# mfkiwl/erlangnetwork-gnsslib-sdr

Hardware: AMD Instinct MI355X
Metric: correlations/sec (1 ms coh) + x real-time, 32-SV L1CA @16.368 Msps (higher is better)
Workload: dtype int8 samples x int8 carrier LUT -> int32 accumulators (exact); NCOs: the reference's fp64 running sums, bit for bit; 1 GPU; BASELINE configs[2]: 32-SV GPS L1CA tracking, 5-tap E/P/L correlators (CORRN=2, CORRD=3), 1 ms coherent, 16.368 Msps int8 IQ, per GPU; channels_per_gpu=32, epochs_per_launch=1000, taps=5, loop=open (frequencies held per launch); see closed_loop (--full), if_broadcast=none (1 GPU)

## Files before the change

erlangnetwork-gnsslib-sdr_amd/csrc/gnsscorr_nco.h:

```cpp
#pragma once

#include <math.h>
#include <stdint.h>
#include <string.h>
#include <type_traits>

#if defined(__HIPCC__)
#define GC_HD __host__ __device__ inline
#define GC_HDM __host__ __device__
#define GC_HD_NOINLINE __host__ __device__ __attribute__((noinline))
#else
#define GC_HD static inline
#define GC_HDM
#define GC_HD_NOINLINE static
#endif
#if defined(__clang__)
#define GC_FP_STRICT _Pragma("clang fp contract(off)")
#else
#define GC_FP_STRICT
#endif

#if defined(__HIP_DEVICE_COMPILE__)
#define GC_DDIV(a, b) __ddiv_rn((a), (b))
#else
// ... 1483 lines not shown
}

GC_HD bool gc_carrier_value_step_one(const GcCarPlan &P, const GcCarStepC &C, double remcarr, int n, int kprem,
                                     double *remcarr_out)
{
    GC_FP_STRICT
    if (C.ex0 == GC_NO_TABLE || n < 1) return false;
    double x = gc_div_y(remcarr * GC_NCO_CDIV, GC_NCO_DPI, P.ydpi);
    if (!gc_one_binade_walk(x, C.s, n, &x)) return false;
    bool held;
    const double p = gc_prem_checked(x, kprem, &held);
    if (!held) return false;
    *remcarr_out = p;
    return true;
}
```

erlangnetwork-gnsslib-sdr_amd/csrc/gnsscorr_plan.hip:

```cpp
#include <cstdlib>
#include <cstddef>
#include <hip/hip_runtime.h>

#include "gnsscorr_internal.h"

namespace {


#define GC_SPEC_WC  9.313225746154785e-10
#define GC_SPEC_WK  9.313225746154785e-10

struct SpecChan {
    GcCodePlan PC;
    GcCarPlan PK;
    GcCarStepC CK;
    double ci, spc, ps, dlen;
    int clen, smax;
    int tmax;
    bool ok;
};

__device__ __forceinline__ void spec_chan_init(SpecChan &C, const GcChan &c, const GcTrkState &s, bool with_prem)
{
    C.ci = __dmul_rn(c.ti, s.codefreq);
// ... 40 lines not shown
            if (!gc_carrier_claims_step<true>(C.PK, C.CK, g0, n, ck, &G)) G = gc_carrier_period_any<GcFillLoop, GcNoEmit, false>(C.PK, g0, n, fill, ne, &tier);
            dk = G - g1;
            dk = dk > 0.5 * GC_NCO_DPI ? dk - GC_NCO_DPI : (dk < -0.5 * GC_NCO_DPI ? dk + GC_NCO_DPI : dk);
            if (!(fabs(dc) < 1.0e300)) dc = 0.0;
            if (!(fabs(dk) < 1.0e300)) dk = 0.0;
        }
    }
    devc[i] = dc;
    devk[i] = dk;
}

#define GC_SPEC_CHUNK 256
__global__ __launch_bounds__(GC_SPEC_CHUNK) void trk_spec_kernel(const GcChan *__restrict__ chan, const GcTrkState *__restrict__ state_in,
                                                                  const double *__restrict__ devc, const double *__restrict__ devk,
                                                                  int *__restrict__ claims_code, int *__restrict__ claims_car,
                                                                  int nch, int nepoch, int e_off)
{
    __shared__ double shc[GC_SPEC_CHUNK], shk[GC_SPEC_CHUNK];
    const int nchunk = (nepoch + GC_SPEC_CHUNK - 1) / GC_SPEC_CHUNK;
    const int ch = blockIdx.x / nchunk, chunk = blockIdx.x - ch * nchunk, tid = threadIdx.x;
    if (ch >= nch) return;
    const int T = e_off + nepoch;
    const int eb = chunk * GC_SPEC_CHUNK + tid;
    const int e = e_off + eb;
    const int base = e_off + chunk * GC_SPEC_CHUNK;
    double pc = 0.0, pk = 0.0;
    for (int j = tid; j < base; j += GC_SPEC_CHUNK) {
        pc += devc[(size_t)ch * T + j];
        pk += devk[(size_t)ch * T + j];
    }
    shc[tid] = pc;
// ... 14 lines not shown
        shc[tid] += ac;
        shk[tid] += ak;
        __syncthreads();
    }
    if (eb >= nepoch) return;
    const double sumc = basec + (tid ? shc[tid - 1] : 0.0), sumk = basek + (tid ? shk[tid - 1] : 0.0);
    const GcTrkState s = state_in[ch];
    SpecChan C;
    spec_chan_init(C, chan[ch], s, false);
    GcCodeClaims cc;
    GcCarClaims ck;
    cc.tag = 0;
    ck.tag = 0;
    cc.n = cc.pad = 0;
    cc.lo = cc.hi = ck.lo = ck.hi = 0.0;
    if (C.ok) {
        double r0, g0;
        int nhat;
        gc_spec_start(s.remcode, s.remcarr, C.ci, C.spc, C.ps, C.dlen, e, &r0, &g0, &nhat);
        const double rt = r0 + sumc, gt = g0 + sumk;
        int ncode = 0;
        bool bracketed = false;
#pragma unroll 1
        for (int att = 0; att < 2 && !bracketed; att++) {
            const double w = att == 0 ? GC_SPEC_WC : GC_SPEC_WC * 0.00390625;
            const double lo = rt - w, hi = rt + w;
            const int nlo = gc_period_nsamp(C.dlen, lo, C.spc), nhi = gc_period_nsamp(C.dlen, hi, C.spc);
            if (!(nlo == nhi && nlo > 0 && nlo <= (1 << 24))) continue;
            double dummy;
            const bool side = (lo - C.PC.smaxci < 0.0) == (hi - C.PC.smaxci < 0.0);
            const bool oklo = gc_code_claims<true>(C.PC, lo, nlo + 2 * C.smax, cc, &dummy);
            const bool okhi = oklo && gc_code_claims<false>(C.PC, hi, nlo + 2 * C.smax, cc, &dummy);
            const bool tailfits = nlo + 2 * C.smax - cc.jsum <= C.tmax;
            if (side && oklo && okhi && tailfits) {
                bracketed = true;
                ncode = nlo;
                cc.tag = 1;
                cc.n = nlo;
                cc.lo = lo;
                cc.hi = hi;
            }
        }
        if (!bracketed) {
            ncode = gc_period_nsamp(C.dlen, rt, C.spc);
            cc.tag = 0;
            if (ncode > 0 && ncode <= (1 << 24)) {
                double dummy;
                cc.tag = (gc_code_claims<true>(C.PC, rt, ncode + 2 * C.smax, cc, &dummy) && ncode + 2 * C.smax - cc.jsum <= C.tmax) ? 3 : 0;
            }
            cc.n = ncode;
            cc.lo = cc.hi = rt;
        }
        const int nk = ncode;
        if (nk > 0 && nk <= (1 << 24)) {
            bool kbr = false;
// ... 19 lines not shown
                ck.tag = ok ? (ck.tag == 2 ? 2 : 3) : 0;
                ck.lo = ck.hi = gt;
            }
            ck.nl = nk;
        }
    }
    const size_t row = (size_t)ch * nepoch + eb;
    int4 *rc = reinterpret_cast<int4 *>(claims_code) + row * (GC_CLAIM_ROW / 4);
    int4 *rk = reinterpret_cast<int4 *>(claims_car) + row * (GC_CLAIM_ROW / 4);
    const int4 *pc4 = reinterpret_cast<const int4 *>(&cc), *pk4 = reinterpret_cast<const int4 *>(&ck);
#pragma unroll
    for (int q = 0; q < GC_CLAIM_ROW / 4; q++) {
        rc[q] = pc4[q];
        rk[q] = pk4[q];
    }
}

__device__ unsigned long long gc_plan_stats[8];

__host__ __device__ inline int plan2_class(double ti, double codefreq, int clen, int smax)
{
    const double ci = ti * codefreq;
    if (!(ci > 0.0) || !gc_fast_has_table(ci)) return -1;
    const int itop = gc_expo(gc_u2d(gc_d2u((double)clen) - 1)) - (gc_expo(ci) + 2);
    if (itop < 7 || itop > 12) return -1;
    if (smax + 1 > GC_CLAIM_TAIL2) return -1;
    return (itop - 7) * 3 + gc_tail_class(smax);
}

#define GC_PLAN_MAXE 4096
__device__ __attribute__((noinline)) void trk_plan_body(const GcChan *__restrict__ chan,
                                                        const GcTrkState *__restrict__ state_in,
                                                        GcTrkState *__restrict__ state_out,
// ... 80 lines not shown
    }
}

__global__ __launch_bounds__(128) void trk_plan_kernel(const GcChan *__restrict__ chan, const GcTrkState *__restrict__ state_in,
                                                       GcTrkState *__restrict__ state_out, GcTrkPlan *__restrict__ plan,
                                                       int nch, int nepoch)
{
    trk_plan_body(chan, state_in, state_out, plan, nch, nepoch);
}

#define GC_P4_BLK 64
struct Plan4Shared {
    int nsh[GC_PLAN_MAXE];
    double vstart[2][GC_P4_BLK];
    unsigned long long vbuff[GC_P4_BLK];
    int prog;
    GcCarPlan pkfull;
};
__shared__ __attribute__((aligned(16))) Plan4Shared g_plan4;

__device__ __forceinline__ int plan2_uni(int v) { return __builtin_amdgcn_readfirstlane(v); }
template <class T>
__device__ __forceinline__ T *plan2_uni(T *p)
{
    const uint64_t u = (uint64_t)p;
    const unsigned lo = (unsigned)__builtin_amdgcn_readfirstlane((int)(unsigned)u);
    const unsigned hi = (unsigned)__builtin_amdgcn_readfirstlane((int)(unsigned)(u >> 32));
    return (T *)(((uint64_t)hi << 32) | lo);
}
__device__ __forceinline__ double plan2_uni(double x)
// ... 7 lines not shown
#define GC_CONST __attribute__((address_space(4)))
typedef int gc_v4i __attribute__((ext_vector_type(4)));
__device__ __forceinline__ GcCodeClaims plan4_code_row(const GC_CONST gc_v4i *r)
{
    const gc_v4i v0 = r[0], v1 = r[1], v2 = r[2], v3 = r[3], v4 = r[4], v5 = r[5];
    GcCodeClaims c;
    c.tag = v0.x; c.i0 = v0.y; c.q = v0.z; c.nl = v0.w;
    c.jsum = v1.x; c.dm[0] = v1.y; c.dm[1] = v1.z; c.dm[2] = v1.w;
    c.dm[3] = v2.x; c.dm[4] = v2.y; c.dm[5] = v2.z; c.dm[6] = v2.w;
    c.dm[7] = v3.x; c.dm[8] = v3.y; c.dm[9] = v3.z; c.dm[10] = v3.w;
    c.dm[11] = v4.x; c.dm[12] = v4.y; c.n = v4.z; c.pad = 0;
    c.lo = gc_u2d(((uint64_t)(unsigned)v5.y << 32) | (unsigned)v5.x);
    c.hi = gc_u2d(((uint64_t)(unsigned)v5.w << 32) | (unsigned)v5.z);
    return c;
}
__device__ __forceinline__ GcCarClaims plan4_car_row(const GC_CONST gc_v4i *r)
{
    const gc_v4i v0 = r[0], v1 = r[1], v2 = r[2], v3 = r[3], v5 = r[5];
    GcCarClaims c;
    c.tag = v0.x; c.nl = v0.y; c.i0 = v0.z; c.nseg = v0.w;
    c.kprem = v1.x; c.dm[0] = v1.y; c.dm[1] = v1.z; c.dm[2] = v1.w;
    c.dm[3] = v2.x; c.dm[4] = v2.y; c.dm[5] = v2.z; c.dm[6] = v2.w;
    c.dm[7] = v3.x; c.dm[8] = v3.y; c.dm[9] = v3.z; c.dm[10] = v3.w;
    c.dm[11] = 0; c.dm[12] = 0; c.pad[0] = 0; c.pad[1] = 0;
    c.lo = gc_u2d(((uint64_t)(unsigned)v5.y << 32) | (unsigned)v5.x);
    c.hi = gc_u2d(((uint64_t)(unsigned)v5.w << 32) | (unsigned)v5.z);
    return c;
}
static_assert(GC_CLAIM_CWIN <= 11, "plan4_car_row reads dm[0..10]");
static_assert(sizeof(GcCodeClaims) == GC_CLAIM_ROW * 4 && sizeof(GcCarClaims) == GC_CLAIM_ROW * 4, "claims rows are GC_CLAIM_ROW ints");
static_assert(offsetof(GcCodeClaims, dm) == 20 && offsetof(GcCarClaims, dm) == 20, "claims layout");
// ... 19 lines not shown
    const int n = plan2_uni(n_);
    const GcCarPlan &PK = g_plan4.pkfull;
    GcFillLanes fill{lane};
    GcNoEmit ne;
    int tier;
    *out = gc_carrier_period_any(PK, remcarr, n, fill, ne, &tier);
    return tier == GC_TIER_PERIOD ? 1 : 2;
}

#ifdef GC_PLAN_PROF
__device__ unsigned long long gc_plan_prof[64 * 16];
#define GC_PP_DECL unsigned long long pp_[7] = {0, 0, 0, 0, 0, 0, 0}
#define GC_PP_T0(v) const unsigned long long v = __builtin_readcyclecounter()
#define GC_PP_ADD(k, v) pp_[k] += __builtin_readcyclecounter() - (v)
#define GC_PP_INC(k) pp_[k] += 1
#define GC_PP_OUT(which) do { if (lane == 0 && blockIdx.x < 64) for (int k_ = 0; k_ < 7; k_++) atomicAdd(&gc_plan_prof[blockIdx.x * 16 + (which) * 8 + k_], pp_[k_]); } while (0)
#else
#define GC_PP_DECL do { } while (0)
#define GC_PP_T0(v) do { } while (0)
#define GC_PP_ADD(k, v) do { } while (0)
#define GC_PP_INC(k) do { } while (0)
#define GC_PP_OUT(which) do { } while (0)
#endif
struct Plan4Job {
    const int4 *claims_code, *claims_car;
    GcTrkPlan *out;
    GcTrkState *state_out;
    GcTrkState s;
    int nepoch, nblk, verify;
};

__device__ __forceinline__ Plan4Job plan4_job(const Plan4Job *J_)
{
    Plan4Job J = *plan2_uni(J_);
    J.claims_code = plan2_uni(J.claims_code);
    J.claims_car = plan2_uni(J.claims_car);
    J.out = plan2_uni(J.out);
    J.state_out = plan2_uni(J.state_out);
    J.nepoch = plan2_uni(J.nepoch);
    J.nblk = plan2_uni(J.nblk);
    J.verify = plan2_uni(J.verify);
    return J;
}

__device__ __forceinline__ int plan4_nb(const Plan4Job &J, int b)
{
    const int left = J.nepoch - b * GC_P4_BLK;
    return left < GC_P4_BLK ? left : GC_P4_BLK;
}

#define GC_GLOBAL __attribute__((address_space(1)))
// ... 23 lines not shown
        c2.tag = 1;
        double rc;
        if (gc_code_claims_step<ITOP, TMAX, false, true>(PC, SC, remcode, n + 2 * smax, c2, &rc)) { *out = rc; return 0; }
    }
    return plan2_code_slow(ci_, clen_, smax_, remcode_, n_, lane, out);
}

__device__ __forceinline__ int plan4_scopy(int x)
{
    int c;
    asm volatile("s_mov_b32 %0, %1" : "=s"(c) : "s"(x));
    return c;
}
__device__ __forceinline__ bool plan4_bcopy(bool x) { return __builtin_amdgcn_readfirstlane(x ? 1 : 0) != 0; }

template <int ITOP, int TMAX>
__device__ __attribute__((noinline)) void plan4_code_wave(double ci_, double spc_, int clen_, int smax_, const Plan4Job *J_, int lane)
{
    const int clen = plan2_uni(clen_), smax = plan2_uni(smax_);
    const double ci = plan2_uni(ci_), spc = plan2_uni(spc_);
    const Plan4Job J = plan4_job(J_);
    const double dlen = (double)clen;
    GcCodePlan PC;
    gc_code_plan_init(PC, ci, clen, smax);
    GcCodeStepC<ITOP> SC;
    gc_code_stepc_init(SC, PC);
    const double yspc = __ddiv_rn(1.0, spc);
    const bool fastdiv = spc > 1e-300 && spc < 1e300 && yspc < 1e300;
    unsigned tally0 = 0, tally1 = 0, tally2 = 0, miss = 0, mism = 0;
    GC_GLOBAL GcTrkPlan *out = (GC_GLOBAL GcTrkPlan *)J.out;
    double remcode = J.s.remcode;
    unsigned long long buffloc = J.s.buffloc;
    GC_PP_DECL;
    GC_PP_T0(ptot_);
    for (int b = 0; b < J.nblk; b++) {
        const int nb = plan4_nb(J, b), e0 = b * GC_P4_BLK;
        const GC_CONST gc_v4i *rows = (const GC_CONST gc_v4i *)J.claims_code + (size_t)e0 * (GC_CLAIM_ROW / 4);
        GcCodeClaims row = plan4_code_row(rows);
        for (int i = 0; i < nb; i++) {
            __builtin_amdgcn_s_waitcnt(0xC07F);
            const double num = __dsub_rn(dlen, remcode);
            double qn = gc_div_y(num, spc, yspc);
            if (__builtin_expect(!fastdiv, 0)) qn = __ddiv_rn(num, spc);
            const int n = plan2_uni((qn > -2147483648.0 && qn < 2147483648.0) ? (int)qn : 0);
            const int tag = row.tag;
            const bool inside = tag == 1 && remcode >= row.lo && remcode <= row.hi && n == row.n;
            double dmd[ITOP + 1];
            const int q = plan4_scopy(row.q), nl = plan4_scopy(row.nl), i0 = plan4_scopy(row.i0);
            const int jsum = plan4_scopy(row.jsum);
#pragma unroll
            for (int k = 0; k <= ITOP; k++) {
                dmd[k] = (double)row.dm[k];
                GC_PIN_V(dmd[k]);
            }
// ... 19 lines not shown
                    const int how = plan4_code_other<ITOP, TMAX>(ci, clen, smax, remcode, n, lane,
                                                                 reinterpret_cast<const GcCodeClaims *>(J.claims_code) + e0 + i, &rs);
                    GC_PP_ADD(1, pslow_);
                    GC_PP_INC(4);
                    tally0 += how == 0 ? 1 : 0;
                    tally1 += how == 1 ? 1 : 0;
                    tally2 += how == 2 ? 1 : 0;
                    mism += (inside_u && how != 0) ? 1 : 0;
                    miss += (!inside_u && claims_u) ? 1 : 0;
                    rc = rs;
                }
                remcode = rc;
            }
            buffloc += (unsigned long long)(long long)n;
        }
        if (lane < nb) {
            GC_GLOBAL GcTrkPlan *o = out + e0 + lane;
            o->buffloc = g_plan4.vbuff[lane];
            o->coff = g_plan4.vstart[0][lane];
            o->carrfreq = J.s.carrfreq;
            o->codefreq = J.s.codefreq;
            o->n = g_plan4.nsh[e0 + lane];
            o->pad = 0;
        }
    }
    GC_PP_ADD(0, ptot_);
    GC_PP_OUT(0);
    if (lane == 0) {
        GC_GLOBAL GcTrkState *so = (GC_GLOBAL GcTrkState *)J.state_out;
        so->carrfreq = J.s.carrfreq;
        so->codefreq = J.s.codefreq;
        so->remcode = remcode;
        so->buffloc = buffloc;
        if (tally0) atomicAdd(&gc_plan_stats[0], (unsigned long long)tally0);
        if (tally1) atomicAdd(&gc_plan_stats[1], (unsigned long long)tally1);
        if (tally2) atomicAdd(&gc_plan_stats[2], (unsigned long long)tally2);
        if (mism) atomicAdd(&gc_plan_stats[6], (unsigned long long)mism);
        if (miss) atomicAdd(&gc_plan_stats[7], (unsigned long long)miss);
    }
}

__device__ __attribute__((noinline)) int plan4_car_other(double ps_, int nsamp_, double remcarr_, int n_, int lane, const GcCarClaims *cl_, double *out)
{
    const GcCarClaims *clp = plan2_uni(cl_);
    const int tag = plan2_uni(clp->tag);
    if (tag != 0) {
        const double ps = plan2_uni(ps_), remcarr = plan2_uni(remcarr_);
        const int n = plan2_uni(n_), nsamp = plan2_uni(nsamp_);
// ... 34 lines not shown
                int tier;
                remcarr = gc_carrier_period_any(PK, remcarr, n, fill, ne, &tier);
                tally1 += tier == GC_TIER_PERIOD ? 1 : 0;
                tally2 += tier == GC_TIER_PERIOD ? 0 : 1;
            }
        }
        if (lane < nb) out[e0 + lane].phi0 = g_plan4.vstart[1][lane];
    }
    if (lane == 0) {
        ((GC_GLOBAL GcTrkState *)J.state_out)->remcarr = remcarr;
        if (tally1) atomicAdd(&gc_plan_stats[4], (unsigned long long)tally1);
        if (tally2) atomicAdd(&gc_plan_stats[5], (unsigned long long)tally2);
    }
}

__device__ __attribute__((noinline)) void plan4_car_wave(double ps_, int nsamp_, const Plan4Job *J_, int lane)
{
    const int nsamp = plan2_uni(nsamp_);
    const double ps = plan2_uni(ps_);
    const Plan4Job J = plan4_job(J_);
    {
        const int nlook = J.nepoch < 16 ? J.nepoch : 16;
        int none = 0;
        for (int e = 0; e < nlook; e++)
            none += ((const GC_CONST int *)J.claims_car)[(size_t)e * GC_CLAIM_ROW] == 0 ? 1 : 0;
        if (none == nlook && nlook >= 8) {
            plan4_car_cert_wave(ps, J_, lane);
            return;
        }
    }
    {
        GcCarPlan full;
        gc_car_plan_init(full, ps);
        if (lane == 0) g_plan4.pkfull = full;
    }
    GcCarPlan PK;
    gc_car_plan_init(PK, ps, false, false);
    GcCarStepC CK;
    gc_car_stepc_init(CK, PK, nsamp + 16);
    const int ilo = plan2_uni(CK.ilo);
    unsigned tally0 = 0, tally1 = 0, tally2 = 0, miss = 0, mism = 0;
    GC_GLOBAL GcTrkPlan *out = (GC_GLOBAL GcTrkPlan *)J.out;
    double remcarr = J.s.remcarr;
    int seen = 0;
    GC_PP_DECL;
    GC_PP_T0(ptot_);
    for (int b = 0; b < J.nblk; b++) {
        const int nb = plan4_nb(J, b), e0 = b * GC_P4_BLK;
        const GC_CONST gc_v4i *rows = (const GC_CONST gc_v4i *)J.claims_car + (size_t)e0 * (GC_CLAIM_ROW / 4);
        GcCarClaims row = plan4_car_row(rows);
        for (int i = 0; i < nb; i++) {
            GC_PP_T0(ptop_);
            if (seen <= e0 + i) {
                GC_PP_T0(pn_);
                while (seen <= e0 + i) {
                    seen = plan2_uni(plan4_progress());
                    if (seen <= e0 + i) __builtin_amdgcn_s_sleep(1);
                }
                GC_PP_ADD(3, pn_);
            }
            const int n = plan2_uni(g_plan4.nsh[e0 + i]);
            __builtin_amdgcn_s_waitcnt(0xC07F);
            const int tag = row.tag;
            const bool inside = tag == 1 && remcarr >= row.lo && remcarr <= row.hi && n == row.nl;
            double dmd[GC_CLAIM_CWIN];
            const int p0 = plan4_scopy(row.i0 - ilo);
            const int plast = plan4_scopy(row.i0 - ilo + row.nseg - 1);
            const int kprem = plan4_scopy(row.kprem);
#pragma unroll
            for (int k = 0; k < GC_CLAIM_CWIN; k++) {
                dmd[k] = (double)row.dm[k];
                GC_PIN_V(dmd[k]);
            }
            const bool inside_u = plan4_bcopy(inside);
            const int tag_u = plan4_scopy(tag);
            __builtin_amdgcn_sched_barrier(0);
            if (i + 1 < nb) row = plan4_car_row(rows + (i + 1) * (GC_CLAIM_ROW / 4));
            __builtin_amdgcn_sched_barrier(0);
            if (lane == 0) g_plan4.vstart[1][i] = remcarr;
            GC_PP_ADD(5, ptop_);
            GC_PP_T0(pstep_);
            if (n > 0 && n <= (1 << 24)) {
                double rp = remcarr;
                bool done = false;
                if (inside_u && !J.verify) {
                    rp = gc_carrier_value_step(PK, CK, remcarr, p0, plast, kprem, dmd);
                    done = true;
                } else if (tag_u == 2) {
                    double r2 = remcarr;
                    done = gc_carrier_value_step_one(PK, CK, remcarr, n, kprem, &r2);
                    rp = done ? r2 : rp;
                }
                if (done) {
                    tally0++;
                } else {
                    double rs;
                    GC_PP_T0(pslow_);
                    const int how = plan4_car_other(ps, nsamp, remcarr, n, lane, reinterpret_cast<const GcCarClaims *>(J.claims_car) + e0 + i, &rs);
                    GC_PP_ADD(1, pslow_);
                    GC_PP_INC(4);
                    tally0 += how == 0 ? 1 : 0;
                    tally1 += how == 1 ? 1 : 0;
                    tally2 += how == 2 ? 1 : 0;
                    mism += (inside_u && how != 0) ? 1 : 0;
                    miss += (!inside_u && tag_u == 1) ? 1 : 0;
                    rp = rs;
                }
                remcarr = rp;
            }
            GC_PP_ADD(6, pstep_);
        }
        if (lane < nb) out[e0 + lane].phi0 = g_plan4.vstart[1][lane];
    }
    GC_PP_ADD(0, ptot_);
    GC_PP_OUT(1);
    if (lane == 0) {
        ((GC_GLOBAL GcTrkState *)J.state_out)->remcarr = remcarr;
        if (tally0) atomicAdd(&gc_plan_stats[3], (unsigned long long)tally0);
        if (tally1) atomicAdd(&gc_plan_stats[4], (unsigned long long)tally1);
        if (tally2) atomicAdd(&gc_plan_stats[5], (unsigned long long)tally2);
        if (mism) atomicAdd(&gc_plan_stats[6], (unsigned long long)mism);
        if (miss) atomicAdd(&gc_plan_stats[7], (unsigned long long)miss);
    }
}

template <int ITOP>
__device__ __forceinline__ void plan4_code_dispatch(int tcls, double ci, double spc, int clen, int smax, const Plan4Job *J, int lane)
{
    if (tcls == 0) plan4_code_wave<ITOP, gc_tail_max(0)>(ci, spc, clen, smax, J, lane);
    else if (tcls == 1) plan4_code_wave<ITOP, gc_tail_max(1)>(ci, spc, clen, smax, J, lane);
    else plan4_code_wave<ITOP, gc_tail_max(2)>(ci, spc, clen, smax, J, lane);
}

__global__ __launch_bounds__(128) void trk_plan4_kernel(const GcChan *__restrict__ chan, const GcTrkState *__restrict__ state_in,
                                                        GcTrkState *__restrict__ state_out, GcTrkPlan *__restrict__ plan,
                                                        int nch, int nepoch, const int *__restrict__ claims_code,
                                                        const int *__restrict__ claims_car, int verify)
{
    const int ch = blockIdx.x, tid = threadIdx.x, lane = tid & 63, wave = tid >> 6;
    if (ch >= nch) return;
    const GcChan c = chan[ch];
    const GcTrkState s = state_in[ch];
    const double ci = __dmul_rn(c.ti, s.codefreq), spc = __ddiv_rn(s.codefreq, c.f_sf), ps = gc_carrier_ps(s.carrfreq, c.ti);
    const int cls = plan2_class(c.ti, s.codefreq, c.clen, c.smax);
    if (cls < 0 || !(ci > 0.0 && ci < (double)c.clen)) {
        trk_plan_body(chan, state_in, state_out, plan, nch, nepoch);
        return;
    }
    const int itop = cls / 3 + 7, tcls = cls % 3;
    constexpr int RW4 = GC_CLAIM_ROW / 4;
    Plan4Job J;
    J.claims_code = reinterpret_cast<const int4 *>(claims_code) + (size_t)ch * nepoch * RW4;
    J.claims_car = reinterpret_cast<const int4 *>(claims_car) + (size_t)ch * nepoch * RW4;
    J.out = plan + (size_t)ch * nepoch;
    J.state_out = state_out + ch;
    J.s = s;
    J.nepoch = nepoch;
    J.nblk = (nepoch + GC_P4_BLK - 1) / GC_P4_BLK;
    J.verify = verify;
    if (tid == 0) g_plan4.prog = 0;
    __syncthreads();
    __builtin_amdgcn_s_setprio(3);
    if (wave == 0) {
        gc_with_itop(itop, [&](auto IT) { plan4_code_dispatch<decltype(IT)::value>(tcls, ci, spc, c.clen, c.smax, &J, lane); return true; });
    } else {
        plan4_car_wave(ps, c.nsamp, &J, lane);
    }
}
// ... 8 lines not shown
    if (hipMemcpyFromSymbol(dst, HIP_SYMBOL(gc_plan_prof), sizeof(unsigned long long) * 64 * 16) != hipSuccess) return -1;
    return 0;
}
#endif

extern "C" int gnsscorr_debug_plan_stats(unsigned long long *dst, int reset)
{
    if (hipMemcpyFromSymbol(dst, HIP_SYMBOL(gc_plan_stats), sizeof(unsigned long long) * 8) != hipSuccess) return -1;
    if (reset) {
        unsigned long long z[8] = {0, 0, 0, 0, 0, 0, 0, 0};
        if (hipMemcpyToSymbol(HIP_SYMBOL(gc_plan_stats), z, sizeof(z)) != hipSuccess) return -1;
    }
    return 0;
}

static bool trk_nospec()
{
    static const bool nospec = getenv("GNSSCORR_TRK_NOSPEC") != nullptr;
    return nospec;
}

size_t gc_trk_spec_ints(size_t units) { return units * (2 * GC_CLAIM_ROW + 8); }

int gc_launch_trk_spec(hipStream_t st, const GcChan *chan, const GcTrkState *state_in, int nch, int nepoch, int *claims,
                       int e_off)
{
    if (!claims || trk_nospec() || nepoch > GC_PLAN_MAXE || e_off < 0 || e_off > nepoch) return 0;
    const size_t units = (size_t)nch * nepoch;
    const int T = e_off + nepoch;
    double *devc = reinterpret_cast<double *>(claims + 2 * units * GC_CLAIM_ROW), *devk = devc + 2 * units;
    hipLaunchKernelGGL(trk_specdev_kernel, dim3((nch * T + 63) / 64), dim3(64), 0, st, chan, state_in, devc, devk, nch, T);
    GC_HIP(hipGetLastError());
    const int nchunk = (nepoch + GC_SPEC_CHUNK - 1) / GC_SPEC_CHUNK;
    hipLaunchKernelGGL(trk_spec_kernel, dim3(nch * nchunk), dim3(GC_SPEC_CHUNK), 0, st, chan, state_in, devc, devk, claims,
                       claims + units * GC_CLAIM_ROW, nch, nepoch, e_off);
    GC_HIP(hipGetLastError());
    return 0;
}

int gc_launch_trk_plan(hipStream_t st, const GcChan *chan, const GcTrkState *state_in, GcTrkState *state_out,
                       GcTrkPlan *plan, int nch, int nepoch, int *claims)
{
    static const int verify = getenv("GNSSCORR_PLAN_VERIFY") ? atoi(getenv("GNSSCORR_PLAN_VERIFY")) : 0;
    const bool batch = claims && !trk_nospec() && nepoch <= GC_PLAN_MAXE;
    if (batch)
        hipLaunchKernelGGL(trk_plan4_kernel, dim3(nch), dim3(128), 0, st, chan, state_in, state_out, plan, nch, nepoch,
                           claims, claims + (size_t)nch * nepoch * GC_CLAIM_ROW, verify);
    else
        hipLaunchKernelGGL(trk_plan_kernel, dim3(nch), dim3(128), 0, st, chan, state_in, state_out, plan, nch, nepoch);
    GC_HIP(hipGetLastError());
    return 0;
}
```

Measured before the change: 266.6 million correlations/s.

## Parallelize plan NCO walk with wave-wide integer prefix scans and precomputed carrier records

The spec kernel now also writes a per-epoch code-scan row: an integer lattice offset and step derived from the bracketing claims. The plan4 code wave uses these rows to advance the code NCO across a whole block of epochs in parallel. A wave prefix sum produces each epoch's start phase and buffer offset, and the serial per-epoch loop runs only from the first epoch that fails validation. The carrier wave precomputes compact per-lane records, including one-binade constants for single-step rows, into shared memory and walks them two at a time. The aim is to shorten the serial dependency chain in the planning kernel, at the cost of extra scratch memory, more bookkeeping and fallback complexity for keeping the fp64 results bit-exact.

```diff
diff --git a/erlangnetwork-gnsslib-sdr_amd/csrc/gnsscorr_nco.h b/erlangnetwork-gnsslib-sdr_amd/csrc/gnsscorr_nco.h
--- a/erlangnetwork-gnsslib-sdr_amd/csrc/gnsscorr_nco.h
+++ b/erlangnetwork-gnsslib-sdr_amd/csrc/gnsscorr_nco.h
@@ -1521,3 +1521,139 @@
     *remcarr_out = p;
     return true;
 }
+
+#define GC_REC_TAG(c)    ((c) & 3)
+#define GC_REC_NMATCH    (1 << 2)
+#define GC_REC_WALK      (1 << 3)
+#define GC_REC_P0(c)     (((c) >> 4) & 15)
+#define GC_REC_PLAST(c)  (((c) >> 8) & 15)
+#define GC_REC_KPREM(c)  (((c) >> 12) & 15)
+#define GC_REC_TIE       (1 << 16)
+#define GC_REC_ONE       (1 << 17)
+#define GC_REC_ROW1      (1 << 18)
+struct GcCarRec {
+    double lo, hi;
+    double dmd[GC_CLAIM_CWIN];
+    int ctl;
+    int key;
+};
+
+GC_HD bool gc_one_binade_consts(int ex, double s, double *d, bool *tie, double *top)
+{
+    GC_FP_STRICT
+    const uint64_t us = gc_d2u(s);
+    const int es = gc_expo(s);
+    *tie = false;
+    if (ex == 0 || ex == 0x7FF || es == 0 || es == 0x7FF) return false;
+    const int et = es + 1075 - ex;
+    if (et >= 1023 + 51) return false;
+    double b = 0.0;
+    if (et >= 1023 - 1) {
+        const double t = gc_u2d((us & 0x800FFFFFFFFFFFFFull) | ((uint64_t)et << 52));
+        b = rint(t);
+        *tie = fabs(t - b) == 0.5;
+    }
+    *d = ldexp(b, ex - 1075);
+    *top = gc_u2d(((uint64_t)ex << 52) | 0x000FFFFFFFFFFFFFull);
+    return true;
+}
+
+GC_HD void gc_car_rec_make(GcCarRec &R, const GcCarClaims &row, int n, int ilo, int ex0, double s, double ydpi)
+{
+    GC_FP_STRICT
+    int tag = row.tag & 3;
+    const int p0 = row.i0 - ilo, plast = p0 + row.nseg - 1;
+    if (tag == 1 && !(p0 >= 0 && plast >= p0 && plast < GC_CLAIM_CWIN)) tag = 3;
+    if ((tag == 1 || tag == 2) && !(row.kprem >= 0 && row.kprem <= GC_CLAIM_PREM)) tag = 3;
+    int ctl = tag | ((row.tag & 3) == 1 ? GC_REC_ROW1 : 0);
+    ctl |= n == row.nl ? GC_REC_NMATCH : 0;
+    ctl |= (n > 0 && n <= (1 << 24)) ? GC_REC_WALK : 0;
+    R.lo = row.lo;
+    R.hi = row.hi;
+    R.key = 0;
+    for (int p = 0; p < GC_CLAIM_CWIN; p++) R.dmd[p] = 0.0;
+    if (tag == 1) {
+        ctl |= (p0 << 4) | (plast << 8) | (row.kprem << 12);
+        for (int p = 0; p < GC_CLAIM_CWIN; p++) R.dmd[p] = (double)row.dm[p];
+    } else if (tag == 2) {
+        ctl |= row.kprem << 12;
+        const double xlo = gc_div_y(row.lo * GC_NCO_CDIV, GC_NCO_DPI, ydpi);
+        const double xhi = gc_div_y(row.hi * GC_NCO_CDIV, GC_NCO_DPI, ydpi);
+        const int klo = (int)(gc_d2u(xlo) >> 52), khi = (int)(gc_d2u(xhi) >> 52);
+        double d, top;
+        bool tie;
+        if (ex0 != GC_NO_TABLE && klo == khi && (klo >> 11) == (int)(gc_d2u(s) >> 63) &&
+            gc_one_binade_consts(klo & 0x7FF, s, &d, &tie, &top)) {
+            ctl |= GC_REC_ONE | (tie ? GC_REC_TIE : 0);
+            R.key = klo;
+            R.dmd[0] = d;
+            R.dmd[1] = top;
+            R.dmd[2] = (double)n;
+        }
+    }
+    R.ctl = ctl;
+}
+
+GC_HD bool gc_carrier_rec_step_one(double ydpi, double remcarr, int key, bool tie, double d, double top, double nd, int kprem,
+                                   double *remcarr_out)
+{
+    GC_FP_STRICT
+    const double x = gc_div_y(remcarr * GC_NCO_CDIV, GC_NCO_DPI, ydpi);
+    const uint64_t ux = gc_d2u(x);
+    if ((int)(ux >> 52) != key) return false;
+    if (tie && (ux & 1)) return false;
+    const double y = fma(nd, d, x);
+    if (!(fabs(y) <= top)) return false;
+    bool held;
+    const double p = gc_prem_checked(y, kprem, &held);
+    if (!held) return false;
+    *remcarr_out = p;
+    return true;
+}
+
+struct GcCodeScanRow {
+    long long Yhat, K;
+    double r1;
+    int valid, pad;
+};
+
+GC_HD double gc_code_scan_head(double remcode, double smaxci, double dlen, bool *neg, int *ecs)
+{
+    GC_FP_STRICT
+    const double cs = remcode - smaxci;
+    *neg = cs < 0.0;
+    *ecs = gc_expo(cs);
+    return cs + dlen;
+}
+
+GC_HD double gc_code_scan_u(double dlen) { return gc_u2d((uint64_t)(gc_expo(gc_u2d(gc_d2u(dlen) - 1)) - 52) << 52); }
+GC_HD double gc_code_scan_invu(double dlen) { return gc_u2d((uint64_t)(2046 - (gc_expo(gc_u2d(gc_d2u(dlen) - 1)) - 52)) << 52); }
+
+GC_HD void gc_code_scan_row(GcCodeScanRow &R, const GcCodePlan &P, double lo, double hi, double r1lo, double r1hi)
+{
+    GC_FP_STRICT
+    R.Yhat = R.K = 0;
+    R.r1 = r1lo;
+    R.valid = R.pad = 0;
+    if (!P.ok || P.it >= P.itop) return;
+    const int etop = gc_expo(P.limtop);
+    bool n0, n1, n2, n3;
+    int e0, e1, e2, e3;
+    const double y0 = gc_code_scan_head(lo, P.smaxci, P.dlen, &n0, &e0), y1 = gc_code_scan_head(hi, P.smaxci, P.dlen, &n1, &e1);
+    const double z0 = gc_code_scan_head(r1lo, P.smaxci, P.dlen, &n2, &e2), z1 = gc_code_scan_head(r1hi, P.smaxci, P.dlen, &n3, &e3);
+    if (!(n0 && n1 && n2 && n3) || e0 != e1 || e2 != e3) return;
+    if (gc_expo(y0) != etop || gc_expo(y1) != etop || gc_expo(z0) != etop || gc_expo(z1) != etop) return;
+    if (!(y0 < P.dlen && y1 < P.dlen && z0 < P.dlen && z1 < P.dlen)) return;
+    const double invu = gc_code_scan_invu(P.dlen);
+    const double k0 = (z0 - y0) * invu, k1 = (z1 - y1) * invu;
+    if (!(k0 == k1) || !(fabs(k0) < 4503599627370496.0) || floor(k0) != k0) return;
+    R.Yhat = (long long)(y0 * invu);
+    R.K = (long long)k0;
+    R.valid = 1;
+}
+
+GC_HD double gc_code_scan_next(double r1, long long Yhat, long long Y, double u)
+{
+    GC_FP_STRICT
+    return r1 + (double)(Y - Yhat) * u;
+}
diff --git a/erlangnetwork-gnsslib-sdr_amd/csrc/gnsscorr_plan.hip b/erlangnetwork-gnsslib-sdr_amd/csrc/gnsscorr_plan.hip
--- a/erlangnetwork-gnsslib-sdr_amd/csrc/gnsscorr_plan.hip
+++ b/erlangnetwork-gnsslib-sdr_amd/csrc/gnsscorr_plan.hip
@@ -78,7 +78,7 @@
 __global__ __launch_bounds__(GC_SPEC_CHUNK) void trk_spec_kernel(const GcChan *__restrict__ chan, const GcTrkState *__restrict__ state_in,
                                                                   const double *__restrict__ devc, const double *__restrict__ devk,
                                                                   int *__restrict__ claims_code, int *__restrict__ claims_car,
-                                                                  int nch, int nepoch, int e_off)
+                                                                  GcCodeScanRow *__restrict__ scan, int nch, int nepoch, int e_off)
 {
     __shared__ double shc[GC_SPEC_CHUNK], shk[GC_SPEC_CHUNK];
     const int nchunk = (nepoch + GC_SPEC_CHUNK - 1) / GC_SPEC_CHUNK;
@@ -123,6 +123,10 @@
     ck.tag = 0;
     cc.n = cc.pad = 0;
     cc.lo = cc.hi = ck.lo = ck.hi = 0.0;
+    GcCodeScanRow srow;
+    srow.Yhat = srow.K = 0;
+    srow.r1 = 0.0;
+    srow.valid = srow.pad = 0;
     if (C.ok) {
         double r0, g0;
         int nhat;
@@ -136,10 +140,10 @@
             const double lo = rt - w, hi = rt + w;
             const int nlo = gc_period_nsamp(C.dlen, lo, C.spc), nhi = gc_period_nsamp(C.dlen, hi, C.spc);
             if (!(nlo == nhi && nlo > 0 && nlo <= (1 << 24))) continue;
-            double dummy;
+            double flo = 0.0, fhi = 0.0;
             const bool side = (lo - C.PC.smaxci < 0.0) == (hi - C.PC.smaxci < 0.0);
-            const bool oklo = gc_code_claims<true>(C.PC, lo, nlo + 2 * C.smax, cc, &dummy);
-            const bool okhi = oklo && gc_code_claims<false>(C.PC, hi, nlo + 2 * C.smax, cc, &dummy);
+            const bool oklo = gc_code_claims<true>(C.PC, lo, nlo + 2 * C.smax, cc, &flo);
+            const bool okhi = oklo && gc_code_claims<false>(C.PC, hi, nlo + 2 * C.smax, cc, &fhi);
             const bool tailfits = nlo + 2 * C.smax - cc.jsum <= C.tmax;
             if (side && oklo && okhi && tailfits) {
                 bracketed = true;
@@ -148,6 +152,7 @@
                 cc.n = nlo;
                 cc.lo = lo;
                 cc.hi = hi;
+                gc_code_scan_row(srow, C.PC, lo, hi, flo, fhi);
             }
         }
         if (!bracketed) {
@@ -197,9 +202,13 @@
         rc[q] = pc4[q];
         rk[q] = pk4[q];
     }
+    scan[row] = srow;
 }
 
 __device__ unsigned long long gc_plan_stats[8];
+#define GC_PLAN_REC_CH 64
+__device__ unsigned long long gc_plan_rec[2 * GC_PLAN_REC_CH];
+__device__ unsigned long long gc_plan_scan[GC_PLAN_REC_CH];
 
 __host__ __device__ inline int plan2_class(double ti, double codefreq, int clen, int smax)
 {
@@ -310,6 +319,7 @@
     int nsh[GC_PLAN_MAXE];
     double vstart[2][GC_P4_BLK];
     unsigned long long vbuff[GC_P4_BLK];
+    GcCarRec rec[GC_P4_BLK];
     int prog;
     GcCarPlan pkfull;
 };
@@ -347,7 +357,8 @@
     c.hi = gc_u2d(((uint64_t)(unsigned)v5.w << 32) | (unsigned)v5.z);
     return c;
 }
-__device__ __forceinline__ GcCarClaims plan4_car_row(const GC_CONST gc_v4i *r)
+template <class RowPtr>
+__device__ __forceinline__ GcCarClaims plan4_car_row(RowPtr r)
 {
     const gc_v4i v0 = r[0], v1 = r[1], v2 = r[2], v3 = r[3], v5 = r[5];
     GcCarClaims c;
@@ -397,16 +408,19 @@
 #define GC_PP_T0(v) const unsigned long long v = __builtin_readcyclecounter()
 #define GC_PP_ADD(k, v) pp_[k] += __builtin_readcyclecounter() - (v)
 #define GC_PP_INC(k) pp_[k] += 1
+#define GC_PP_ADDN(k, n) pp_[k] += (n)
 #define GC_PP_OUT(which) do { if (lane == 0 && blockIdx.x < 64) for (int k_ = 0; k_ < 7; k_++) atomicAdd(&gc_plan_prof[blockIdx.x * 16 + (which) * 8 + k_], pp_[k_]); } while (0)
 #else
 #define GC_PP_DECL do { } while (0)
 #define GC_PP_T0(v) do { } while (0)
 #define GC_PP_ADD(k, v) do { } while (0)
 #define GC_PP_INC(k) do { } while (0)
+#define GC_PP_ADDN(k, n) do { } while (0)
 #define GC_PP_OUT(which) do { } while (0)
 #endif
 struct Plan4Job {
     const int4 *claims_code, *claims_car;
+    const GcCodeScanRow *scan;
     GcTrkPlan *out;
     GcTrkState *state_out;
     GcTrkState s;
@@ -418,6 +432,7 @@
     Plan4Job J = *plan2_uni(J_);
     J.claims_code = plan2_uni(J.claims_code);
     J.claims_car = plan2_uni(J.claims_car);
+    J.scan = plan2_uni(J.scan);
     J.out = plan2_uni(J.out);
     J.state_out = plan2_uni(J.state_out);
     J.nepoch = plan2_uni(J.nepoch);
@@ -471,6 +486,64 @@
 }
 __device__ __forceinline__ bool plan4_bcopy(bool x) { return __builtin_amdgcn_readfirstlane(x ? 1 : 0) != 0; }
 
+__device__ __forceinline__ long long plan4_wscan(long long v, int lane)
+{
+#pragma unroll
+    for (int d = 1; d < 64; d <<= 1) {
+        const long long t = __shfl_up(v, d, 64);
+        v += lane >= d ? t : 0;
+    }
+    return v;
+}
+__device__ __forceinline__ double plan4_lane_d(double x, int l) { return plan2_uni(__shfl(x, l, 64)); }
+__device__ __forceinline__ long long plan4_lane_ll(long long x, int l)
+{
+    const long long v = __shfl(x, l, 64);
+    const unsigned lo = (unsigned)__builtin_amdgcn_readfirstlane((int)(unsigned)(unsigned long long)v);
+    const unsigned hi = (unsigned)__builtin_amdgcn_readfirstlane((int)(unsigned)((unsigned long long)v >> 32));
+    return (long long)(((unsigned long long)hi << 32) | lo);
+}
+__device__ __forceinline__ int plan4_lane_i(int x, int l) { return plan2_uni(__shfl(x, l, 64)); }
+
+struct Plan4ScanK {
+    double smaxci, dlen, spc, yspc, u, invu;
+    bool fastdiv;
+};
+struct Plan4ScanLane {
+    long long Yhat, K;
+    double r1, lo, hi;
+    int valid, tag, rown;
+    double rem, nxt;
+    long long bl;
+    int n;
+    bool inside;
+};
+
+__device__ __forceinline__ int plan4_scan_round(Plan4ScanLane &L, const Plan4ScanK &K, int start, int nb, int lane, double rem0, unsigned long long buff0)
+{
+    bool neg;
+    int ecs;
+    const long long Y0 = (long long)(gc_code_scan_head(rem0, K.smaxci, K.dlen, &neg, &ecs) * K.invu);
+    const bool act = lane >= start && lane < nb;
+    const bool rowok = act && L.tag == 1 && L.valid != 0;
+    const long long k = rowok ? L.K : 0;
+    const long long Y = Y0 + plan4_wscan(k, lane) - k;
+    L.nxt = gc_code_scan_next(L.r1, L.Yhat, Y, K.u);
+    const double prev = __shfl_up(L.nxt, 1, 64);
+    L.rem = lane == start ? rem0 : prev;
+    const double num = __dsub_rn(K.dlen, L.rem);
+    double qn = gc_div_y(num, K.spc, K.yspc);
+    if (__builtin_expect(!K.fastdiv, 0)) qn = __ddiv_rn(num, K.spc);
+    L.n = (qn > -2147483648.0 && qn < 2147483648.0) ? (int)qn : 0;
+    L.inside = L.tag == 1 && L.rem >= L.lo && L.rem <= L.hi && L.n == L.rown;
+    const bool ok = rowok && L.inside && L.n > 0 && L.n <= (1 << 24);
+    const unsigned long long bad = __ballot(act && !ok);
+    const int f = bad ? (int)__builtin_ctzll(bad) : nb;
+    const long long nn = act ? (long long)L.n : 0;
+    L.bl = (long long)buff0 + plan4_wscan(nn, lane) - nn;
+    return plan2_uni(f);
+}
+
 template <int ITOP, int TMAX>
 __device__ __attribute__((noinline)) void plan4_code_wave(double ci_, double spc_, int clen_, int smax_, const Plan4Job *J_, int lane)
 {
@@ -485,16 +558,90 @@
     const double yspc = __ddiv_rn(1.0, spc);
     const bool fastdiv = spc > 1e-300 && spc < 1e300 && yspc < 1e300;
     unsigned tally0 = 0, tally1 = 0, tally2 = 0, miss = 0, mism = 0;
+    unsigned scanned = 0;
     GC_GLOBAL GcTrkPlan *out = (GC_GLOBAL GcTrkPlan *)J.out;
     double remcode = J.s.remcode;
     unsigned long long buffloc = J.s.buffloc;
+    Plan4ScanK SK;
+    SK.smaxci = PC.smaxci;
+    SK.dlen = dlen;
+    SK.spc = spc;
+    SK.yspc = yspc;
+    SK.u = gc_code_scan_u(dlen);
+    SK.invu = gc_code_scan_invu(dlen);
+    SK.fastdiv = fastdiv;
+    const bool scan_on = J.scan != nullptr && PC.ok;
     GC_PP_DECL;
     GC_PP_T0(ptot_);
     for (int b = 0; b < J.nblk; b++) {
         const int nb = plan4_nb(J, b), e0 = b * GC_P4_BLK;
         const GC_CONST gc_v4i *rows = (const GC_CONST gc_v4i *)J.claims_code + (size_t)e0 * (GC_CLAIM_ROW / 4);
-        GcCodeClaims row = plan4_code_row(rows);
-        for (int i = 0; i < nb; i++) {
+        Plan4ScanLane L = {};
+        int ifrom = 0;
+        if (scan_on) {
+            const int el = e0 + (lane < nb ? lane : nb - 1);
+            const GC_GLOBAL gc_v4i *sr = (const GC_GLOBAL gc_v4i *)J.scan + (size_t)el * 2;
+            const GC_GLOBAL gc_v4i *cr = (const GC_GLOBAL gc_v4i *)J.claims_code + (size_t)el * (GC_CLAIM_ROW / 4);
+            const gc_v4i s0 = sr[0], s1 = sr[1], c0 = cr[0], c4 = cr[4], c5 = cr[5];
+            L.Yhat = (long long)(((unsigned long long)(unsigned)s0.y << 32) | (unsigned)s0.x);
+            L.K = (long long)(((unsigned long long)(unsigned)s0.w << 32) | (unsigned)s0.z);
+            L.r1 = gc_u2d(((uint64_t)(unsigned)s1.y << 32) | (unsigned)s1.x);
+            L.valid = s1.z;
+            L.tag = c0.x;
+            L.rown = c4.z;
+            L.lo = gc_u2d(((uint64_t)(unsigned)c5.y << 32) | (unsigned)c5.x);
+            L.hi = gc_u2d(((uint64_t)(unsigned)c5.w << 32) | (unsigned)c5.z);
+        }
+        if (scan_on && !J.verify) {
+            int start = 0, empty = 0;
+            while (start < nb) {
+                const int f = plan4_scan_round(L, SK, start, nb, lane, remcode, buffloc);
+                if (lane >= start && lane < f) {
+                    g_plan4.vstart[0][lane] = L.rem;
+                    g_plan4.vbuff[lane] = (unsigned long long)L.bl;
+                    g_plan4.nsh[e0 + lane] = L.n;
+                }
+                tally0 += (unsigned)(f - start);
+                scanned += (unsigned)(f - start);
+                if (f >= nb) {
+                    remcode = plan4_lane_d(L.nxt, nb - 1);
+                    buffloc = (unsigned long long)plan4_lane_ll(L.bl + (long long)L.n, nb - 1);
+                    start = nb;
+                    break;
+                }
+                remcode = plan4_lane_d(L.rem, f);
+                buffloc = (unsigned long long)plan4_lane_ll(L.bl, f);
+                empty = f == start ? empty + 1 : 0;
+                if (empty >= 2) {
+                    start = f;
+                    break;
+                }
+                const int n = plan4_lane_i(L.n, f);
+                const bool inside_u = plan4_lane_i(L.inside ? 1 : 0, f) != 0, claims_u = plan4_lane_i(L.tag, f) == 1;
+                if (lane == 0) {
+                    g_plan4.vstart[0][f] = remcode;
+                    g_plan4.vbuff[f] = buffloc;
+                    g_plan4.nsh[e0 + f] = n;
+                }
+                if (n > 0 && n <= (1 << 24)) {
+                    double rs;
+                    const int how = plan4_code_other<ITOP, TMAX>(ci, clen, smax, remcode, n, lane,
+                                                                 reinterpret_cast<const GcCodeClaims *>(J.claims_code) + e0 + f, &rs);
+                    GC_PP_INC(4);
+                    tally0 += how == 0 ? 1 : 0;
+                    tally1 += how == 1 ? 1 : 0;
+                    tally2 += how == 2 ? 1 : 0;
+                    mism += (inside_u && how != 0) ? 1 : 0;
+                    miss += (!inside_u && claims_u) ? 1 : 0;
+                    remcode = rs;
+                }
+                buffloc += (unsigned long long)(long long)n;
+                start = f + 1;
+            }
+            ifrom = start;
+        }
+        GcCodeClaims row = plan4_code_row(rows + (ifrom < nb ? ifrom : 0) * (GC_CLAIM_ROW / 4));
+        for (int i = ifrom; i < nb; i++) {
             __builtin_amdgcn_s_waitcnt(0xC07F);
             const double num = __dsub_rn(dlen, remcode);
             double qn = gc_div_y(num, spc, yspc);
@@ -544,6 +691,24 @@
             }
             buffloc += (unsigned long long)(long long)n;
         }
+        if (scan_on && J.verify) {
+            int start = 0;
+            while (start < nb) {
+                const double rem0 = plan2_uni(g_plan4.vstart[0][start]);
+                const unsigned long long b0 = (unsigned long long)plan4_lane_ll((long long)g_plan4.vbuff[start], 0);
+                const int f = plan4_scan_round(L, SK, start, nb, lane, rem0, b0);
+                const int last = f < nb ? f : nb - 1;
+                const int li = lane < nb ? lane : 0;
+                const bool differs = lane >= start && lane <= last &&
+                                     (gc_d2u(L.rem) != gc_d2u(g_plan4.vstart[0][li]) || (unsigned long long)L.bl != g_plan4.vbuff[li] ||
+                                      L.n != g_plan4.nsh[e0 + li]);
+                mism += (unsigned)__popcll(__ballot(differs));
+                scanned += (unsigned)(f - start);
+                if (f >= nb) mism += gc_d2u(plan4_lane_d(L.nxt, nb - 1)) != gc_d2u(remcode) ? 1 : 0;
+                start = f + 1;
+            }
+        }
+        if (lane == 0) plan4_publish(e0 + nb);
         if (lane < nb) {
             GC_GLOBAL GcTrkPlan *o = out + e0 + lane;
             o->buffloc = g_plan4.vbuff[lane];
@@ -562,6 +727,7 @@
         so->codefreq = J.s.codefreq;
         so->remcode = remcode;
         so->buffloc = buffloc;
+        if (scanned && blockIdx.x < GC_PLAN_REC_CH) atomicAdd(&gc_plan_scan[blockIdx.x], (unsigned long long)scanned);
         if (tally0) atomicAdd(&gc_plan_stats[0], (unsigned long long)tally0);
         if (tally1) atomicAdd(&gc_plan_stats[1], (unsigned long long)tally1);
         if (tally2) atomicAdd(&gc_plan_stats[2], (unsigned long long)tally2);
@@ -626,6 +792,107 @@
     }
 }
 
+__device__ __attribute__((noinline)) int plan4_car_one(double s_, int ex0_, double remcarr_, int n_, int ctl_, int key_, double d_, double top_,
+                                                       double nd_, int verify_, double *out)
+{
+    const int verify = plan2_uni(verify_);
+    const double s = plan2_uni(s_), remcarr = plan2_uni(remcarr_), d = plan2_uni(d_), top = plan2_uni(top_), nd = plan2_uni(nd_);
+    const int ex0 = plan2_uni(ex0_), n = plan2_uni(n_), ctl = plan2_uni(ctl_), key = plan2_uni(key_);
+    GcCarPlan P;
+    P.ydpi = 1.0 / GC_NCO_DPI;
+    GcCarStepC C;
+    C.s = s;
+    C.ex0 = ex0;
+    double r = remcarr, r2 = remcarr;
+    const bool done = gc_carrier_value_step_one(P, C, remcarr, n, GC_REC_KPREM(ctl), &r);
+    int bad = 0;
+    if (verify && (ctl & GC_REC_ONE)) {
+        const bool done2 = gc_carrier_rec_step_one(P.ydpi, remcarr, key, (ctl & GC_REC_TIE) != 0, d, top, nd, GC_REC_KPREM(ctl), &r2);
+        bad = (done2 && (!done || gc_d2u(r2) != gc_d2u(r))) ? 2 : 0;
+    }
+    if (done) *out = r;
+    return (done ? 1 : 0) | bad;
+}
+
+__device__ __forceinline__ void plan4_rec_load(GcCarRec &R, int i)
+{
+    const GcCarRec &r = g_plan4.rec[i];
+    R.lo = r.lo;
+    R.hi = r.hi;
+#pragma unroll
+    for (int p = 0; p < GC_CLAIM_CWIN; p++) R.dmd[p] = r.dmd[p];
+    R.ctl = r.ctl;
+    R.key = r.key;
+}
+
+struct Plan4CarRun {
+    double remcarr, phi;
+    unsigned recwin, recone;
+    unsigned tally0, tally1, tally2, miss, mism, slow;
+    unsigned long long slowclk;
+};
+
+#ifdef GC_PLAN_PROF
+#define GC_PP_SLOW0(v) const unsigned long long v = __builtin_readcyclecounter()
+#define GC_PP_SLOW1(S, v) (S).slowclk += __builtin_readcyclecounter() - (v)
+#else
+#define GC_PP_SLOW0(v) do { } while (0)
+#define GC_PP_SLOW1(S, v) do { } while (0)
+#endif
+
+__device__ __forceinline__ void plan4_car_period(Plan4CarRun &S, const GcCarRec &R, const GcCarPlan &PK, const GcCarStepC &CK, double ps, int nsamp,
+                                                 const Plan4Job &J, int e, int i, int lane)
+{
+    const int ctl = plan2_uni(R.ctl);
+    const int tag = GC_REC_TAG(ctl);
+    const double remcarr = S.remcarr;
+    const bool inside_u = plan4_bcopy(remcarr >= R.lo && remcarr <= R.hi) && (ctl & (3 | GC_REC_NMATCH)) == (1 | GC_REC_NMATCH);
+    S.phi = lane == i ? remcarr : S.phi;
+    if (!(ctl & GC_REC_WALK)) return;
+    double rp = remcarr;
+    bool done = false;
+    if (inside_u && !J.verify) {
+        rp = gc_carrier_value_step(PK, CK, remcarr, GC_REC_P0(ctl), GC_REC_PLAST(ctl), GC_REC_KPREM(ctl), R.dmd);
+        done = true;
+        S.recwin++;
+    } else if (tag == 2) {
+        if ((ctl & GC_REC_ONE) && !J.verify) {
+            double r2 = remcarr;
+            done = plan4_bcopy(gc_carrier_rec_step_one(PK.ydpi, remcarr, plan2_uni(R.key), (ctl & GC_REC_TIE) != 0, R.dmd[0], R.dmd[1], R.dmd[2],
+                                                       GC_REC_KPREM(ctl), &r2));
+            rp = done ? r2 : rp;
+            S.recone += done ? 1 : 0;
+        }
+        if (!done) {
+            double r1;
+            const int n = plan2_uni(g_plan4.nsh[e]);
+            GC_PP_SLOW0(pone_);
+            const int how = plan4_car_one(CK.s, CK.ex0, remcarr, n, ctl, R.key, R.dmd[0], R.dmd[1], R.dmd[2], J.verify, &r1);
+            GC_PP_SLOW1(S, pone_);
+            done = (how & 1) != 0;
+            S.slow++;
+            S.tally0 += done ? 1 : 0;
+            S.mism += (how & 2) ? 1 : 0;
+            if (done) rp = r1;
+        }
+    }
+    if (!done) {
+        double rs;
+        const int n = plan2_uni(g_plan4.nsh[e]);
+        GC_PP_SLOW0(pother_);
+        const int how = plan4_car_other(ps, nsamp, remcarr, n, lane, reinterpret_cast<const GcCarClaims *>(J.claims_car) + e, &rs);
+        GC_PP_SLOW1(S, pother_);
+        S.slow++;
+        S.tally0 += how == 0 ? 1 : 0;
+        S.tally1 += how == 1 ? 1 : 0;
+        S.tally2 += how == 2 ? 1 : 0;
+        S.mism += (inside_u && how != 0) ? 1 : 0;
+        S.miss += (!inside_u && (ctl & GC_REC_ROW1)) ? 1 : 0;
+        rp = rs;
+    }
+    S.remcarr = rp;
+}
+
 __device__ __attribute__((noinline)) void plan4_car_wave(double ps_, int nsamp_, const Plan4Job *J_, int lane)
 {
     const int nsamp = plan2_uni(nsamp_);
@@ -650,89 +917,68 @@
     gc_car_plan_init(PK, ps, false, false);
     GcCarStepC CK;
     gc_car_stepc_init(CK, PK, nsamp + 16);
-    const int ilo = plan2_uni(CK.ilo);
-    unsigned tally0 = 0, tally1 = 0, tally2 = 0, miss = 0, mism = 0;
+    const int ilo = plan2_uni(CK.ilo), ex0 = plan2_uni(CK.ex0);
     GC_GLOBAL GcTrkPlan *out = (GC_GLOBAL GcTrkPlan *)J.out;
-    double remcarr = J.s.remcarr;
+    Plan4CarRun S;
+    S.remcarr = J.s.remcarr;
+    S.phi = 0.0;
+    S.recwin = S.recone = S.tally0 = S.tally1 = S.tally2 = S.miss = S.mism = S.slow = 0;
+    S.slowclk = 0;
     int seen = 0;
     GC_PP_DECL;
     GC_PP_T0(ptot_);
     for (int b = 0; b < J.nblk; b++) {
         const int nb = plan4_nb(J, b), e0 = b * GC_P4_BLK;
-        const GC_CONST gc_v4i *rows = (const GC_CONST gc_v4i *)J.claims_car + (size_t)e0 * (GC_CLAIM_ROW / 4);
-        GcCarClaims row = plan4_car_row(rows);
-        for (int i = 0; i < nb; i++) {
-            GC_PP_T0(ptop_);
-            if (seen <= e0 + i) {
-                GC_PP_T0(pn_);
-                while (seen <= e0 + i) {
-                    seen = plan2_uni(plan4_progress());
-                    if (seen <= e0 + i) __builtin_amdgcn_s_sleep(1);
-                }
-                GC_PP_ADD(3, pn_);
-            }
-            const int n = plan2_uni(g_plan4.nsh[e0 + i]);
-            __builtin_amdgcn_s_waitcnt(0xC07F);
-            const int tag = row.tag;
-            const bool inside = tag == 1 && remcarr >= row.lo && remcarr <= row.hi && n == row.nl;
-            double dmd[GC_CLAIM_CWIN];
-            const int p0 = plan4_scopy(row.i0 - ilo);
-            const int plast = plan4_scopy(row.i0 - ilo + row.nseg - 1);
-            const int kprem = plan4_scopy(row.kprem);
-#pragma unroll
-            for (int k = 0; k < GC_CLAIM_CWIN; k++) {
-                dmd[k] = (double)row.dm[k];
-                GC_PIN_V(dmd[k]);
-            }
-            const bool inside_u = plan4_bcopy(inside);
-            const int tag_u = plan4_scopy(tag);
+        GC_PP_T0(ptop_);
+        const int el = e0 + (lane < nb ? lane : nb - 1);
+        const GcCarClaims row = plan4_car_row((const GC_GLOBAL gc_v4i *)J.claims_car + (size_t)el * (GC_CLAIM_ROW / 4));
+        if (seen < e0 + nb) {
+            GC_PP_T0(pn_);
+            while (seen < e0 + nb) {
+                seen = plan2_uni(plan4_progress());
+                if (seen < e0 + nb) __builtin_amdgcn_s_sleep(1);
+            }
+            GC_PP_ADD(3, pn_);
+        }
+        {
+            GcCarRec mine;
+            gc_car_rec_make(mine, row, g_plan4.nsh[el], ilo, ex0, CK.s, PK.ydpi);
+            if (lane < nb) g_plan4.rec[lane] = mine;
+        }
+        asm volatile("" ::: "memory");
+        __builtin_amdgcn_wave_barrier();
+        GC_PP_ADD(5, ptop_);
+        GC_PP_T0(pstep_);
+        GcCarRec A, B;
+        plan4_rec_load(A, 0);
+        for (int i = 0; i < nb; i += 2) {
+            plan4_rec_load(B, i + 1 < nb ? i + 1 : i);
             __builtin_amdgcn_sched_barrier(0);
-            if (i + 1 < nb) row = plan4_car_row(rows + (i + 1) * (GC_CLAIM_ROW / 4));
+            plan4_car_period(S, A, PK, CK, ps, nsamp, J, e0 + i, i, lane);
+            if (i + 1 >= nb) break;
+            plan4_rec_load(A, i + 2 < nb ? i + 2 : i + 1);
             __builtin_amdgcn_sched_barrier(0);
-            if (lane == 0) g_plan4.vstart[1][i] = remcarr;
-            GC_PP_ADD(5, ptop_);
-            GC_PP_T0(pstep_);
-            if (n > 0 && n <= (1 << 24)) {
-                double rp = remcarr;
-                bool done = false;
-                if (inside_u && !J.verify) {
-                    rp = gc_carrier_value_step(PK, CK, remcarr, p0, plast, kprem, dmd);
-                    done = true;
-                } else if (tag_u == 2) {
-                    double r2 = remcarr;
-                    done = gc_carrier_value_step_one(PK, CK, remcarr, n, kprem, &r2);
-                    rp = done ? r2 : rp;
-                }
-                if (done) {
-                    tally0++;
-                } else {
-                    double rs;
-                    GC_PP_T0(pslow_);
-                    const int how = plan4_car_other(ps, nsamp, remcarr, n, lane, reinterpret_cast<const GcCarClaims *>(J.claims_car) + e0 + i, &rs);
-                    GC_PP_ADD(1, pslow_);
-                    GC_PP_INC(4);
-                    tally0 += how == 0 ? 1 : 0;
-                    tally1 += how == 1 ? 1 : 0;
-                    tally2 += how == 2 ? 1 : 0;
-                    mism += (inside_u && how != 0) ? 1 : 0;
-                    miss += (!inside_u && tag_u == 1) ? 1 : 0;
-                    rp = rs;
-                }
-                remcarr = rp;
-            }
-            GC_PP_ADD(6, pstep_);
-        }
-        if (lane < nb) out[e0 + lane].phi0 = g_plan4.vstart[1][lane];
+            plan4_car_period(S, B, PK, CK, ps, nsamp, J, e0 + i + 1, i + 1, lane);
+        }
+        GC_PP_ADD(6, pstep_);
+        if (lane < nb) out[e0 + lane].phi0 = S.phi;
     }
     GC_PP_ADD(0, ptot_);
+    GC_PP_ADDN(1, S.slowclk);
+    GC_PP_ADDN(4, S.slow);
     GC_PP_OUT(1);
     if (lane == 0) {
-        ((GC_GLOBAL GcTrkState *)J.state_out)->remcarr = remcarr;
-        if (tally0) atomicAdd(&gc_plan_stats[3], (unsigned long long)tally0);
-        if (tally1) atomicAdd(&gc_plan_stats[4], (unsigned long long)tally1);
-        if (tally2) atomicAdd(&gc_plan_stats[5], (unsigned long long)tally2);
-        if (mism) atomicAdd(&gc_plan_stats[6], (unsigned long long)mism);
-        if (miss) atomicAdd(&gc_plan_stats[7], (unsigned long long)miss);
+        ((GC_GLOBAL GcTrkState *)J.state_out)->remcarr = S.remcarr;
+        S.tally0 += S.recwin + S.recone;
+        if (blockIdx.x < GC_PLAN_REC_CH) {
+            if (S.recwin) atomicAdd(&gc_plan_rec[blockIdx.x * 2], (unsigned long long)S.recwin);
+            if (S.recone) atomicAdd(&gc_plan_rec[blockIdx.x * 2 + 1], (unsigned long long)S.recone);
+        }
+        if (S.tally0) atomicAdd(&gc_plan_stats[3], (unsigned long long)S.tally0);
+        if (S.tally1) atomicAdd(&gc_plan_stats[4], (unsigned long long)S.tally1);
+        if (S.tally2) atomicAdd(&gc_plan_stats[5], (unsigned long long)S.tally2);
+        if (S.mism) atomicAdd(&gc_plan_stats[6], (unsigned long long)S.mism);
+        if (S.miss) atomicAdd(&gc_plan_stats[7], (unsigned long long)S.miss);
     }
 }
 
@@ -747,7 +993,7 @@
 __global__ __launch_bounds__(128) void trk_plan4_kernel(const GcChan *__restrict__ chan, const GcTrkState *__restrict__ state_in,
                                                         GcTrkState *__restrict__ state_out, GcTrkPlan *__restrict__ plan,
                                                         int nch, int nepoch, const int *__restrict__ claims_code,
-                                                        const int *__restrict__ claims_car, int verify)
+                                                        const int *__restrict__ claims_car, const GcCodeScanRow *__restrict__ scan, int verify)
 {
     const int ch = blockIdx.x, tid = threadIdx.x, lane = tid & 63, wave = tid >> 6;
     if (ch >= nch) return;
@@ -764,6 +1010,7 @@
     Plan4Job J;
     J.claims_code = reinterpret_cast<const int4 *>(claims_code) + (size_t)ch * nepoch * RW4;
     J.claims_car = reinterpret_cast<const int4 *>(claims_car) + (size_t)ch * nepoch * RW4;
+    J.scan = scan ? scan + (size_t)ch * nepoch : nullptr;
     J.out = plan + (size_t)ch * nepoch;
     J.state_out = state_out + ch;
     J.s = s;
@@ -802,13 +1049,35 @@
     return 0;
 }
 
+extern "C" int gnsscorr_debug_plan_rec(unsigned long long *dst, int reset)
+{
+    if (hipMemcpyFromSymbol(dst, HIP_SYMBOL(gc_plan_rec), sizeof(unsigned long long) * 2 * GC_PLAN_REC_CH) != hipSuccess) return -1;
+    if (reset) {
+        unsigned long long z[2 * GC_PLAN_REC_CH] = {0};
+        if (hipMemcpyToSymbol(HIP_SYMBOL(gc_plan_rec), z, sizeof(z)) != hipSuccess) return -1;
+    }
+    return 0;
+}
+
+extern "C" int gnsscorr_debug_plan_scan(unsigned long long *dst, int reset)
+{
+    if (hipMemcpyFromSymbol(dst, HIP_SYMBOL(gc_plan_scan), sizeof(unsigned long long) * GC_PLAN_REC_CH) != hipSuccess) return -1;
+    if (reset) {
+        unsigned long long z[GC_PLAN_REC_CH] = {0};
+        if (hipMemcpyToSymbol(HIP_SYMBOL(gc_plan_scan), z, sizeof(z)) != hipSuccess) return -1;
+    }
+    return 0;
+}
+
 static bool trk_nospec()
 {
     static const bool nospec = getenv("GNSSCORR_TRK_NOSPEC") != nullptr;
     return nospec;
 }
 
-size_t gc_trk_spec_ints(size_t units) { return units * (2 * GC_CLAIM_ROW + 8); }
+size_t gc_trk_spec_ints(size_t units) { return units * (2 * GC_CLAIM_ROW + 8 + 8); }
+static_assert(sizeof(GcCodeScanRow) == 32 && ((2 * GC_CLAIM_ROW + 8) * 4) % 32 == 0, "scan rows lie 32-byte aligned behind the deviations");
+static GcCodeScanRow *trk_scan_rows(int *claims, size_t units) { return reinterpret_cast<GcCodeScanRow *>(claims + units * (2 * GC_CLAIM_ROW + 8)); }
 
 int gc_launch_trk_spec(hipStream_t st, const GcChan *chan, const GcTrkState *state_in, int nch, int nepoch, int *claims,
                        int e_off)
@@ -821,7 +1090,7 @@
     GC_HIP(hipGetLastError());
     const int nchunk = (nepoch + GC_SPEC_CHUNK - 1) / GC_SPEC_CHUNK;
     hipLaunchKernelGGL(trk_spec_kernel, dim3(nch * nchunk), dim3(GC_SPEC_CHUNK), 0, st, chan, state_in, devc, devk, claims,
-                       claims + units * GC_CLAIM_ROW, nch, nepoch, e_off);
+                       claims + units * GC_CLAIM_ROW, trk_scan_rows(claims, units), nch, nepoch, e_off);
     GC_HIP(hipGetLastError());
     return 0;
 }
@@ -833,7 +1102,8 @@
     const bool batch = claims && !trk_nospec() && nepoch <= GC_PLAN_MAXE;
     if (batch)
         hipLaunchKernelGGL(trk_plan4_kernel, dim3(nch), dim3(128), 0, st, chan, state_in, state_out, plan, nch, nepoch,
-                           claims, claims + (size_t)nch * nepoch * GC_CLAIM_ROW, verify);
+                           claims, claims + (size_t)nch * nepoch * GC_CLAIM_ROW,
+                           (const GcCodeScanRow *)trk_scan_rows(claims, (size_t)nch * nepoch), verify);
     else
         hipLaunchKernelGGL(trk_plan_kernel, dim3(nch), dim3(128), 0, st, chan, state_in, state_out, plan, nch, nepoch);
     GC_HIP(hipGetLastError());
```

Result: faster. 307.4 million correlations/s, median of 6 (+15.3%).
